# latentnetworks/vimure

Hardware: AMD Instinct MI355X
Metric: CAVI iterations/sec (L=4 N=2000 M=200 K=2 synthetic, mutuality on) (higher is better)
Workload: dtype f64

## Files before the change

### include/vimure_hip.h

```cpp
#ifndef VIMURE_HIP_H
#define VIMURE_HIP_H

#include <stdint.h>

#ifdef __cplusplus
extern "C" {
#endif

typedef struct vmr_ctx* vmr_handle;

enum {
  VMR_OK = 0,
  VMR_EINVAL = -1,
  VMR_EHIP = -2,
  VMR_ENAN = -3,
  VMR_ESTATE = -4
};

enum { VMR_STEP_GAMMA = 0, VMR_STEP_PHI = 1, VMR_STEP_RHO = 2, VMR_STEP_NU = 3 };

enum { VMR_READ_RHO_MAX = 0, VMR_READ_RHO_MEAN = 1, VMR_READ_THRESHOLD = 2 };

enum {
  VMR_KERNEL_GAMMA_MASK = 0,
// ... 157 lines not shown
int vmr_get_geometric(vmr_handle h, double* g_theta, double* g_lambda, double* g_nu, double* g_nu_cache);

int vmr_sync(vmr_handle h);

int vmr_profile(vmr_handle h, int enable);
int vmr_profile_read(vmr_handle h, int kernel_class, double* total_ms, int64_t* launches);

int vmr_kernel_bytes(vmr_handle h, int kernel_class, double* bytes);

int vmr_data_format(vmr_handle h, int* sparse, uint64_t* nnz);

int vmr_mask_format(vmr_handle h, int* lists, uint64_t* listed);

int vmr_sweep_shape(vmr_handle h, int* passes, int* lds_levels, uint64_t* far_reports);

int vmr_generate_y(int device, int L, int N, int K, int C, const double* w, const int32_t* grp, uint64_t seed, uint8_t* Y_dev);
int vmr_generate_x(int device, int L, int N, int M, const uint8_t* Y_dev, const double* lam_dev, const double* theta, double eta,
                   double lambda_diff, uint64_t seed, int self_reporter, uint8_t* X_dev);

const char* vmr_version(void);

#ifdef __cplusplus
}
#endif
#endif
```

### vimure_amd/_lib.py

```python
import ctypes as C
import os

HERE = os.path.dirname(os.path.abspath(__file__))
LIB_PATH = os.environ.get("VMR_LIB", os.path.join(HERE, "libvimure_hip.so"))

VMR_OK, VMR_EINVAL, VMR_EHIP, VMR_ENAN, VMR_ESTATE = 0, -1, -2, -3, -4
STEP_GAMMA, STEP_PHI, STEP_RHO, STEP_NU = 0, 1, 2, 3
KERNEL_GAMMA_MASK, KERNEL_GAMMA_COUNTS, KERNEL_PHI, KERNEL_RHO, KERNEL_ELBO, KERNEL_FINALIZE, KERNEL_RHO_ELBO, KERNEL_RHO_NOSTORE = range(8)
READ_RHO_MAX, READ_RHO_MEAN, READ_THRESHOLD = 0, 1, 2
PPC_NSTAT = 6
TRIAD_NSTAT = 6
TRIAD_NAMES = ["transitive", "cyclic", "two_paths", "triangles_u", "wedges_u", "edges_u"]
EDGE_REPORTED, EDGE_INFERRED = 1, 2
SCORE_RHO1, SCORE_PROB = 0, 1
SCORE_NCONF, SCORE_NSUM, SCORE_MAX_THR = 5, 4, 4096
RT_NCOUNT, RT_NSUM = 7, 3
RT_COUNT_NAMES = ["n_scope", "n_rep", "total", "n_inferred", "hits", "mutual", "n_out"]
RT_SUM_NAMES = ["exp_ties", "exp_hits", "exp_total"]
HO_NSUM, HO_NCOUNT = 4, 4
HO_SUM_NAMES = ["logp", "sq_err", "total", "exp_total"]
HO_COUNT_NAMES = ["n", "n_pos", "n_inf", "n_in_mask"]
RS_REPORTS, RS_OMISSIONS = 1, 2
RS_NSUM, RS_NCOUNT, RS_MAX_EDGES = 4, 4, 4096
RS_SUM_NAMES = ["logp", "sq_err", "total", "exp_total"]
# ... 58 lines not shown
    "vmr_report_scores_size": (C.c_int, [C.c_void_p, C.c_int, C.c_void_p, C.c_void_p, C.c_double, C.c_int, C.c_double, C.POINTER(C.c_uint64)]),
    "vmr_report_scores": (C.c_int, [C.c_void_p, C.c_int, C.c_void_p, C.c_void_p, C.c_double, C.c_int, C.c_double, C.c_int, C.c_void_p]
                          + [C.c_void_p] * 4 + [C.c_uint64] + [C.c_void_p] * 8 + [C.c_int]),
    "vmr_reporter_influence_size": (C.c_int, [C.c_void_p, C.c_int] + [C.c_void_p] * 4 + [C.c_double, C.c_int, C.c_double, C.c_int, C.c_double,
                                              C.POINTER(C.c_uint64)]),
    "vmr_reporter_influence": (C.c_int, [C.c_void_p, C.c_int] + [C.c_void_p] * 4 + [C.c_double, C.c_int, C.c_double, C.c_int, C.c_double,
                                         C.c_int, C.c_void_p] + [C.c_void_p] * 3 + [C.c_uint64] + [C.c_void_p] * 9 + [C.c_int]),
    "vmr_snapshot": (C.c_int, [C.c_void_p]),
    "vmr_restore": (C.c_int, [C.c_void_p]),
    "vmr_profile": (C.c_int, [C.c_void_p, C.c_int]),
    "vmr_profile_read": (C.c_int, [C.c_void_p, C.c_int, _dp, C.POINTER(C.c_int64)]),
    "vmr_kernel_bytes": (C.c_int, [C.c_void_p, C.c_int, _dp]),
    "vmr_data_format": (C.c_int, [C.c_void_p, C.POINTER(C.c_int), C.POINTER(C.c_uint64)]),
    "vmr_mask_format": (C.c_int, [C.c_void_p, C.POINTER(C.c_int), C.POINTER(C.c_uint64)]),
    "vmr_sweep_shape": (C.c_int, [C.c_void_p, C.POINTER(C.c_int), C.POINTER(C.c_int), C.POINTER(C.c_uint64)]),
    "vmr_generate_y": (C.c_int, [C.c_int, C.c_int, C.c_int, C.c_int, C.c_int, C.c_void_p, C.c_void_p, C.c_uint64, C.c_void_p]),
    "vmr_generate_x": (C.c_int, [C.c_int, C.c_int, C.c_int, C.c_int, C.c_void_p, C.c_void_p, C.c_void_p, C.c_double, C.c_double,
                                 C.c_uint64, C.c_int, C.c_void_p]),
    "vmr_version": (C.c_char_p, []),
}

_lib = None


def load():
    global _lib
    if _lib is not None:
        return _lib
    if not os.path.exists(LIB_PATH):
        raise RuntimeError(
# ... 16 lines not shown
```

### vimure_amd/csrc/sorted_lists.hip

```cpp
#include "sweep_sl.h"

__global__ __launch_bounds__(256) void k_sl_keys(const unsigned* __restrict__ cnt, unsigned* __restrict__ keys, unsigned* __restrict__ vals, size_t T) {
  for (size_t t = (size_t)blockIdx.x * 256 + threadIdx.x; t < T; t += (size_t)gridDim.x * 256) { keys[t] = cnt[t]; vals[t] = (unsigned)t; }
}
__global__ __launch_bounds__(256) void k_sl_level_keys(unsigned* __restrict__ keys, const unsigned* __restrict__ rpl, const unsigned* __restrict__ E,
                                                       size_t T, unsigned rows0, int nb) {
  for (size_t t = (size_t)blockIdx.x * 256 + threadIdx.x; t < T; t += (size_t)gridDim.x * 256) {
    const unsigned r0 = rpl[t], n = rpl[t + 1] - r0;
    unsigned n1 = 0;
    for (unsigned r = 0; r < n; ++r) n1 += SL_YM(E[(size_t)r0 + r]) >= rows0 ? 1u : 0u;
    keys[t] = (n << nb) | n1;
  }
}
__global__ __launch_bounds__(256) void k_sl_steps(const unsigned* __restrict__ keys_sorted, const unsigned* __restrict__ vals_sorted,
                                                  unsigned* __restrict__ sz, unsigned* __restrict__ perm, size_t T, size_t NS, int nb) {
  for (size_t q = (size_t)blockIdx.x * 256 + threadIdx.x; q < NS * 64; q += (size_t)gridDim.x * 256) {
    perm[q] = q < T ? vals_sorted[q] : 0xffffffffu;
    if ((q & 63) == 0) sz[q >> 6] = 64u * (keys_sorted[q] >> nb);
  }
  if (blockIdx.x == 0 && threadIdx.x == 0) sz[NS] = 0u;
}
__global__ __launch_bounds__(256) void k_sl_place(const unsigned* __restrict__ perm, const unsigned* __restrict__ rpl ,
                                                  const unsigned* __restrict__ rsl, const unsigned* __restrict__ Ein,
                                                  unsigned* __restrict__ Eout, const unsigned* __restrict__ Ein2, unsigned* __restrict__ Eout2,
// ... 77 lines not shown
  CKS(hipMalloc(&h->perm, (size_t)L * NS * 64 * 4));
  CKS(hipMalloc(&h->sy, (size_t)L * NS * 4));
  size_t tb = 0;
  int bits = 1;
  while (bits < 32 && (1ull << bits) <= (unsigned long long)g.M) ++bits;
  const bool level_keys_ok = !wide && g.mut && 2 * bits <= 30 && !h->opt.no_level_sort;
  CKS(hipcub::DeviceRadixSort::SortPairsDescending(nullptr, tb, keys, keys2, vals, vals2, (int)T, 0, level_keys_ok ? 2 * bits : bits, h->stream));
  CKS(hipMalloc(&tmp, tb ? tb : 8));
  const unsigned tgrid = (unsigned)std::min<size_t>(8192, (T + 255) / 256), sgrid = (unsigned)std::min<size_t>(8192, (NS + 3) / 4);
  if (!etmp_all) {
    unsigned long long nlmax = 0;
    for (int l = 0; l < L; ++l) nlmax = std::max(nlmax, nl[l]);
    CKS(hipMalloc(&etmp, ((size_t)nlmax + 64) * 4));
    if (wide) CKS(hipMalloc(&etmp2, ((size_t)nlmax + 64) * 4));
  }
  unsigned long long off1 = 0;
  for (int l = 0; l < L; ++l) {
    unsigned* rpl = rp + (size_t)l * n;
    unsigned* rsl = h->rs + (size_t)l * (NS + 1);
    const bool by_level = level_keys_ok && (double)nl[l] > (double)SL_PF * (double)T;
    const int nb = by_level ? bits : 0;
    int rc;
    hipLaunchKernelGGL(k_sl_keys, dim3(tgrid), dim3(256), 0, h->stream, rpl, keys, vals, T);
    if (by_level) {
      if ((rc = scan_u32(h, rpl, bsum, n))) { cleanup(); return rc; }
      if (!etmp_all) (*fill)(l, rpl, etmp, etmp2);
      hipLaunchKernelGGL(k_sl_level_keys, dim3(tgrid), dim3(256), 0, h->stream, keys, rpl, etmp_all ? etmp_all + off1 : etmp, T, (unsigned)g.Mp, nb);
    }
    CKS(hipcub::DeviceRadixSort::SortPairsDescending(tmp, tb, keys, keys2, vals, vals2, (int)T, 0, bits + nb, h->stream));
    hipLaunchKernelGGL(k_sl_steps, dim3((unsigned)std::min<size_t>(8192, (NS * 64 + 255) / 256)), dim3(256), 0, h->stream, keys2, vals2, rsl,
                       h->perm + (size_t)l * NS * 64, T, NS, nb);
    CKS(hipGetLastError());
    if ((rc = scan_u32(h, rsl, bsum, NS + 1)) || (!by_level && (rc = scan_u32(h, rpl, bsum, n)))) { cleanup(); return rc; }
    off1 += nl[l];
  }
// ... 52 lines not shown
```

### vimure_amd/csrc/sweep_sl.h

```cpp
#ifndef VMR_SWEEP_SL_H
#define VMR_SWEEP_SL_H

#include "vmr_internal.h"
#include <functional>

#define SL_YM(e) ((e) & 0xfffffu)
#define SL_INR(e) (((e) >> 20) & 1u)
#define SL_X(e) ((e) >> 21)
#define SL_XMAX 2047u
#define SL_YM_ROWS (1u << 20)
#define SL_PF 8
#ifndef SL_PFW
#define SL_PFW 8
#endif
constexpr int sl_pf(int K) { return K <= 2 ? SL_PF : SL_PFW; }
#define SL_SLACK (64 * 64)

struct SlArgs {
  const unsigned* E; const unsigned* rs; const unsigned long long* ebase; const unsigned* perm;
  const unsigned* sy;
  const uint8_t* cls;
  const unsigned* Qt;
  const uint64_t* Rb; const unsigned* rq; const unsigned short* Rm; const unsigned long long* rbase;
  const unsigned* rm2;
// ... 2 lines not shown
  int Gl;
  int do_hist;
  int yt, hc;
  int sum_a;
  double* nu_acc; double* elbo_dev; int commit_nu;
  int nu_stale;
  unsigned long long* det;
  int lp0;
  int farl;
  double* h0s;
  const unsigned* x0p;
  int lv0r;
  const unsigned* Ez;
  int elbo_cur;
  const double* lpd; const double* lpb;
#ifdef SL_DEBUG
  unsigned long long* dbg_t;
#endif
};

struct SlShape { int tpb, yt, hc; size_t smem; };
struct SlUnit { SlArgs a; Geo g; int blk0, nblk; };

#ifndef SL_LIGHT_UPD_K
#define SL_LIGHT_UPD_K 2
#endif
constexpr bool sl_light(int K, bool elbo, bool allfull, bool update) { return !elbo && allfull && (K <= SL_LIGHT_UPD_K || (!update && K <= 4)); }
#ifndef SL_ELBO3_K
#define SL_ELBO3_K 2
#endif
// ... 32 lines not shown
```

### vimure_amd/csrc/sweep_sl.hip

```cpp
#include "sweep_sl.h"

#ifndef VMR_K
#error "compile with -DVMR_K=<number of categories>"
#endif
#ifndef SL_WPE
#define SL_WPE sl_wpe(2, false, true)
#endif

template <int K>
struct StepIn {
  double v[K];
  double w[K];
  unsigned cls, qt, tie;
  unsigned x0;
  unsigned e[sl_pf(K)];
};

template <int R> struct RC { static constexpr int value = R; };
template <class V> __device__ __forceinline__ const V* at_bytes(const V* p, unsigned off) {
  return reinterpret_cast<const V*>(reinterpret_cast<const char*>(p) + off);
}
template <class V> __device__ __forceinline__ V* at_bytes(V* p, unsigned off) {
  return reinterpret_cast<V*>(reinterpret_cast<char*>(p) + off);
}
// ... 1 lines not shown
  double r = __builtin_amdgcn_rcp(d);
  r = fma(fma(-d, r, 1.0), r, r);
  return fma(fma(-d, r, 1.0), r, r);
}
#define SL_INL __attribute__((always_inline))
#ifndef SL_BATCH2
#define SL_BATCH2 8
#endif
template <int K> struct Batch { static constexpr int value = K <= 2 ? SL_BATCH2 : (K <= 4 ? 4 : 2); };

template <int K, bool UPDATE, bool ELBO, bool ALLFULL, bool STORE = true, bool DET = false, bool LPD = false>
__device__ __forceinline__ void sweep_body(const SlArgs& a, const Geo& g, const unsigned bx, const unsigned gx) {
  extern __shared__ __align__(16) unsigned char smem[];
  constexpr int PFK = sl_pf(K);
  constexpr bool LV0 = !UPDATE && !ELBO && !DET;
  constexpr bool LV0R = UPDATE && K >= 3;
  const int tid = threadIdx.x, lane = tid & 63, nthr = (int)blockDim.x;
  const int wv = __builtin_amdgcn_readfirstlane(tid >> 6), nw = nthr >> 6;
  const int Mp = g.Mp;
  const unsigned ytm = UPDATE ? (unsigned)a.yt * (unsigned)Mp : 0u;
  const unsigned hcm = a.do_hist ? (unsigned)a.hc * (unsigned)Mp : 0u;
  size_t off = 0;
  double* F = reinterpret_cast<double*>(smem + off); off += (size_t)ytm * K * 8;
  const int nHc = (int)hcm * K;
  double* Hc = reinterpret_cast<double*>(smem + off); off += (size_t)nHc * 8;
  double* Gth = reinterpret_cast<double*>(smem + off); off += (size_t)Mp * 8;
  double* Lth = reinterpret_cast<double*>(smem + off); off += UPDATE ? (size_t)Mp * 8 : 0;
  double* As = reinterpret_cast<double*>(smem + off); off += a.sum_a ? (size_t)Mp * K * 8 : 0;
  double* wsum = reinterpret_cast<double*>(smem + off); off += (size_t)g.W * 8;
  double* red = reinterpret_cast<double*>(smem + off); off += 16 * 8;
// ... 1 lines not shown
  double* lt = reinterpret_cast<double*>(smem + off); off += ELBO ? 256 * 8 : 0;
  double* EthL = reinterpret_cast<double*>(smem + off); off += a.rq ? (size_t)Mp * 8 : 0;
  const ParOff o = par_off(g.L, g.Mp, g.K);
  const int l = (int)bx / a.Gl, gb = (int)bx - l * a.Gl;
#ifdef SL_DEBUG
  unsigned long long* dbt = a.dbg_t ? a.dbg_t + ((size_t)bx * nw + wv) * 8 : nullptr;
  if (dbt && lane == 0) dbt[0] = wall_clock64();
#endif
  const size_t T = (size_t)g.N * g.N;
  const long long NS = (long long)((T + 63) / 64);
  const double gnu = a.par[o.sc + ((UPDATE || a.elbo_cur) ? SC_G_NU : SC_G_NU_STALE)];
  bool gz = false;
  for (int m = tid; m < Mp; m += nthr) {
    const double gv = a.par[o.G_th + (size_t)l * Mp + m];
    Gth[m] = gv;
    if (LV0 || LV0R) gz = gz || (m < g.M && gv == 0.0);
    if (UPDATE) Lth[m] = a.par[o.l_th + (size_t)l * Mp + m];
  }
  for (int q = tid; q < nHc; q += nthr) Hc[q] = 0.0;
  if (a.sum_a) for (int q = tid; q < Mp * K; q += nthr) As[q] = 0.0;
  if (a.rq) for (int m = tid; m < Mp; m += nthr) EthL[m] = m < g.M ? a.par[o.E_th + (size_t)l * Mp + m] : 0.0;
  if (UPDATE || ELBO) sp_math_tables(xt, lt, tid, nthr, ELBO);
  const double* lut = a.lutg + (size_t)l * g.W * 256;
  for (int w = tid; w < g.W; w += nthr) {
    double v = 0.0;
    for (int n = 0; n < 16; ++n) v += lut[(w * 16 + n) * 16 + 15];
    wsum[w] = v;
  }
  double Ela[K], Gla[K], Lla[K];
#pragma unroll
  for (int k = 0; k < K; ++k) { Ela[k] = a.par[o.E_la + l * K + k]; Gla[k] = a.par[o.G_la + l * K + k]; Lla[k] = a.par[o.l_la + l * K + k]; if (LV0 || LV0R) gz = gz || Gla[k] == 0.0; }
  const double eps = g.eps;
  const double sc_h = DET ? __builtin_amdgcn_ldexp(1.0, g.det_sh) : 0.0;
  const double sc_a = DET ? __builtin_amdgcn_ldexp(1.0, g.det_sha) : 0.0;
  auto fxm = [](double v, double scale) SL_INL -> unsigned long long {
    return (unsigned long long)(__double_as_longlong(fma(v, scale, 6755399441055744.0)) - 0x4338000000000000ll);
  };
  auto lds_add = [&](double* p, double v, double scale) SL_INL {
    if (DET) atomicAdd(reinterpret_cast<unsigned long long*>(p), fxm(v, scale)); else atomicAdd(p, v);
  };
  const float rcp_mp = 1.0f / (float)Mp, hrcp_mp = 0.5f * rcp_mp;
  auto row_level = [&](unsigned ym) SL_INL -> unsigned { return (unsigned)__builtin_fmaf((float)ym, rcp_mp, hrcp_mp); };
  const double lp0_0 = log(1.0 + eps), lp0_k = log(eps);
  double e_lin = 0.0, e_q = 0.0, e_log = 0.0;
  double accF[K], acc0[K];
#pragma unroll
// ... 81 lines not shown
  };

  if (s < NS) {
    ea = rsl[s];
    R = (int)((rsl[s + 1] - ea) >> 6);
    ymax = syl[s];
    fetch_range(sn < NS ? sn : s);
    fetch_tie(P, s);
    fetch_ent(P, ea, RC<PFK>{});
  }
#ifdef SL_DEBUG
  if (dbt && lane == 0) dbt[4] = wall_clock64();
#endif
  __builtin_amdgcn_s_waitcnt(0x0F70);
  bool lv0_off = false;
  if (LV0 || LV0R) lv0_off = __syncthreads_or(gz ? 1 : 0) != 0;
  else __syncthreads();
#ifdef SL_DEBUG
  if (dbt && lane == 0) dbt[5] = wall_clock64();
#endif
  const double gnu_f = a.par[o.sc + (a.nu_stale ? SC_G_NU_STALE : SC_G_NU)];
  if (UPDATE) {
    for (int q = tid; q < (int)ytm; q += nthr) {
      const int y = q / Mp, m = q - y * Mp;
#pragma unroll
      for (int k = 0; k < K; ++k) F[q * K + k] = (m < g.M) ? f_entry(g.mut, Lth[m], Gth[m], Lla[k], Gla[k], gnu_f, y) : 0.0;
    }
    __syncthreads();
  }
  double Tfull = 0.0;
  for (int w = 0; w < g.W; ++w) Tfull += wsum[w];
// ... 128 lines not shown
      if (ELBO) {
#pragma unroll
        for (int u = 0; u < LG; ++u) if (j0 + u < NP) {
          const double term = (double)SL_X(e[j0 + u]) * log_tab(in_[u], lt);
          if (DET) ie_log += det_fx(term, g.det_shr); else e_log += term;
        }
        __builtin_amdgcn_sched_barrier(0);
      }
    }
  };
  auto deficit = [&](unsigned ent, double dfc) SL_INL {
    lds_add(&Hc[SL_YM(ent)], (double)SL_X(ent) * dfc, sc_h);
  };
  auto compute = [&](auto rct, const StepIn<K>& cur, const size_t row0, const bool act, const unsigned ea_c, const int Rr, const unsigned sy_word) SL_INL {
    const unsigned ymax = sy_word & 0xffffu, nf = a.farl ? sy_word >> 16 : 0x7fffffffu;
    const unsigned n1 = (LV0 && a.h0s && !lv0_off) ? sy_word >> 16 : 0x7fffffffu;
    constexpr int RCT = decltype(rct)::value;
    constexpr int NP = RCT < 0 ? PFK : RCT;
    const unsigned cls = cur.cls, qt = cur.qt, tie = cur.tie;
    const unsigned* pe = El + ea_c;
    auto rounds = [&](auto gbc, auto&& use, const int Rr) SL_INL {
      constexpr int GB = decltype(gbc)::value;
      unsigned rg[PFK];
#pragma unroll
      for (int i = 0; i < PFK; ++i) rg[i] = i < Rr ? cur.e[i] : 0u;
      for (int j0 = 0; j0 < Rr; j0 += PFK) {
#pragma unroll
        for (int gi = 0; gi < PFK; gi += GB) {
          unsigned c[GB];
#pragma unroll
          for (int u = 0; u < GB; ++u) {
// ... 144 lines not shown
      if (irr && lane == 0) tick[1] = 1u;
      if (!ELBO && a.do_hist == 1 && act && (ALLFULL || cls == 1u)) {
#pragma unroll
        for (int k = 0; k < K; ++k) { if (DET) iaccF[k] += fxm(r[k], sc_a); else accF[k] += r[k]; }
      }
      if (!ALLFULL && !ELBO && a.sum_a) add_lists(tie, act && cls == 2u, r);
    }
    if (ELBO) {
#pragma unroll
      for (int k = 0; k < K; ++k) { const double ek = exp_tab(r[k], xt); er[0] = fma(ek, Gla[k], er[0]); er[1] += ek; }
    }
#ifdef SL_DEBUG
    if (g.dbg & 32) {} else
#endif
    if (a.do_hist || ELBO) {
      if (RCT >= 0) {
        walk2_near(cur.e, RC<NP>{}, r, er);
        if (irr) {
#pragma unroll
          for (int j = 0; j < NP; ++j) deficit(cur.e[j], dfc);
        }
      } else {
        const bool skip0 = LV0 && a.x0p != nullptr && a.do_hist == 1 && n1 != 0x7fffffffu && !irr;
        const int Rw = skip0 ? min(Rr, (int)n1) : Rr;
        double sx0 = skip0 ? (double)cur.x0 : 0.0;
        rounds(RC<1>{}, [&](const unsigned (&c1)[1], const unsigned j) SL_INL {
          const unsigned c = c1[0], ym = SL_YM(c), x = SL_X(c);
          const bool far_round = j < nf && lim2 != 0xffffffffu;
          const bool fr = far_round && ym >= hcm;
          const double dx = (double)x;
          if (LV0 && a.do_hist && j >= n1) {
            sx0 += dx;
            if (irr) lds_add(&Hc[ym], dx * dfc, sc_h);
          } else if (a.do_hist) {
            if (!fr) {
              if (!(skip0 && ym < (unsigned)Mp)) {
#pragma unroll
                for (int k = 1; k < K; ++k) lds_add(&Hc[(unsigned)k * hcm + ym], dx * r[k], sc_h);
              }
              if (irr) lds_add(&Hc[ym], dx * dfc, sc_h);
            }
            if (far_round && !a.farl && __any(fr)) {
              if (fr && x != 0u) {
                if (DET) {
                  unsigned long long* d0 = a.det;
                  asm volatile("" : "+s"(d0));
                  unsigned long long* d = d0 + (size_t)l * g.Y * Mp * K + (size_t)ym * K;
#pragma unroll
                  for (int k = 1; k < K; ++k) atomicAdd(&d[k], fxm((double)x * r[k], sc_h));
                  if (dfc != 0.0) atomicAdd(&d[0], fxm((double)x * dfc, sc_h));
                } else {
                  double* d = Hl + (size_t)ym * K;
#pragma unroll
                  for (int k = 1; k < K; ++k) atomicAdd(&d[k], (double)x * r[k]);
                  if (dfc != 0.0) atomicAdd(&d[0], (double)x * dfc);
                }
              }
              asm volatile("" ::: "memory");
            }
          }
          if (ELBO) { const double term = (double)x * log_tab(elbo_inner(c, er), lt); if (DET) ie_log += det_fx(term, g.det_shr); else e_log += term; }
        }, Rw);
        if (LV0 && a.h0s && a.do_hist == 1 && act) {
#pragma unroll
          for (int k = 1; k < K; ++k) acc0[k] = fma(r[k], sx0, acc0[k]);
        }
      }
    }
    if (ELBO && act) {
      double sr = 0.0, se = 0.0, en = 0.0;
#pragma unroll
      for (int k = 0; k < K; ++k) {
        sr += r[k]; se += r[k] * Ela[k];
        en += r[k] * cur.v[k] - r[k] * log_tab(r[k] + eps, lt);
      }
      if (DET) { ie_lin += det_fx(en - se * Tt, g.det_shr); if (Ql) ie_q += det_fx(sr * (double)qt, g.det_shr); }
      else { e_lin += en - se * Tt; if (Ql) e_q += sr * (double)qt; }
    }
// ... 44 lines not shown
      case 3: run(RC<3>{}); break;
      case 4: run(RC<4>{}); break;
      case 5: run(RC<5>{}); break;
      case 6: run(RC<6>{}); break;
      case 7: run(RC<7>{}); break;
      default: run(RC<8>{}); break;
    }
  }

#ifdef SL_DEBUG
  if (dbt && lane == 0) dbt[2] = wall_clock64();
#endif
  const bool nu_here = a.nu_acc && a.do_hist == 1;
  if (nu_here) asm volatile("s_waitcnt vmcnt(0)" ::: "memory");
  __syncthreads();
  if (nu_here) {
    double a0p = 0.0;
    for (int q = (tick[1] ? 0 : (int)hcm) + tid; q < nHc; q += nthr) {
      const double v = DET ? det_back(reinterpret_cast<const unsigned long long*>(Hc)[q], g.det_sh) : Hc[q];
      if (v != 0.0) {
        const int k = q / (int)hcm;
        const unsigned ym = (unsigned)(q - k * (int)hcm);
        a0p += ((k ? w2_at(ym, k) : 0.0) - w2_at(ym, 0)) * v;
      }
    }
    a0p = block_sum_n(a0p, red);
    if (tid == 0) {
      if (DET) atomicAdd(&det_R()[4], det_fx(a0p, g.det_sh)); else atomicAdd(&a.nu_acc[0], a0p);
    }
  }
// ... 267 lines not shown
```

### vimure_amd/csrc/vimure_hip.hip

```cpp
#include "vmr_internal.h"
#include "sweep_sl.h"
#include "sweep_gen.h"
#include "sample_draw.h"

thread_local std::string g_create_err;



template <int SH>
__device__ __forceinline__ unsigned nz_flags16(uint4 v) {
  const unsigned M = 0x7f7f7f7fu;
  unsigned t0 = ((v.x & M) + M) | v.x, t1 = ((v.y & M) + M) | v.y;
  unsigned t2 = ((v.z & M) + M) | v.z, t3 = ((v.w & M) + M) | v.w;
  unsigned f = (t0 >> (7 - SH)) & (0x01010101u << SH);
  f |= (t1 >> (6 - SH)) & (0x02020202u << SH);
  f |= (t2 >> (5 - SH)) & (0x04040404u << SH);
  f |= (t3 >> (4 - SH)) & (0x08080808u << SH);
  return f;
}
__device__ __forceinline__ void flag_pos(int bit, int& chunk, int& byte) {
  const int lo = bit & 31;
  chunk = ((bit >> 5) << 1) | ((lo >> 2) & 1);
  byte = ((lo & 3) << 2) | (lo >> 3);
}
// ... 1556 lines not shown
  if (update && !g.two_pass) n += shmem_hc(g);
  if (elbo) n += (size_t)g.Mp * 8 + (size_t)g.nt * 4;
  return n + 16;
}

#define SP_LDS_MAX (160 * 1024)

static SlShape sl_shape(const vmr_ctx* h, bool update, bool elbo, bool hist) {
  const Geo& g = h->g;
  SlShape s{std::max(64, std::min((update || elbo) ? h->sp_tpb : h->st_tpb, sl_tpb_max(g.K, elbo, h->all_full != 0, update)) & ~63), update ? g.yt : 0, hist ? g.hc : 0, 0};
  auto bytes = [&]() { return sl_smem(g, s.yt, s.hc, update, elbo, hist); };
  while (bytes() > SP_LDS_MAX && (s.yt > 0 || s.hc > 0)) { if (s.yt >= s.hc && s.yt > 0) --s.yt; else --s.hc; }
  s.smem = bytes();
  return s;
}
static SlArgs sl_args(const vmr_ctx* h, const SlShape& sh, int do_hist, int sum_a = 0) {
  return SlArgs{h->E, h->rs, h->ebase, h->perm, h->sy, h->cls_p, h->Qt_p, h->Rb, h->rq, h->Rm, h->rbase, h->rm2, h->rho, h->logpr, h->par, h->slotR,
                h->lutg, h->Hg, h->slotF, h->slotA, 1, do_hist, sh.yt, sh.hc, sum_a, nullptr, nullptr, 0, 0, nullptr, h->lp0 ? 1 : 0, h->g.farl, (do_hist == 1 && h->g.two_pass && sh.hc >= 1) ? h->h0s : nullptr, (do_hist == 1 && h->g.two_pass && sh.hc >= 1 && h->h0s) ? h->x0p : nullptr,
                (h->h0s && h->g.two_pass && !h->opt.no_lv0r) ? 1 : 0, h->E + h->n_slots, 0, h->lpd, h->lpb};
}
static int sl_launch(vmr_ctx* h, int mode, const SlShape& sh, SlArgs& a) {
  sl_launch_fn fn = vmr_sl_launcher(h->g.K);
  if (!fn) return fail(h, VMR_EINVAL, "this build of libvimure_hip.so holds no sweep kernel for this K");
  return fn(h, mode, sh, a);
}

#ifdef VMR_DEV
#define DISPATCH_K(K_, ...)                         \
  switch (K_) {                                     \
    case 2: { constexpr int KK = 2; __VA_ARGS__; } break; \
    default: break;                                 \
  }
#else
#define DISPATCH_K(K_, ...)                         \
// ... 12 lines not shown
  switch (PF_) {                                                      \
    case 4: { constexpr int PP = 4; DISPATCH_K(K_, __VA_ARGS__); } break;   \
    case 8: { constexpr int PP = 8; DISPATCH_K(K_, __VA_ARGS__); } break;   \
    default: { constexpr int PP = 12; DISPATCH_K(K_, __VA_ARGS__); } break; \
  }



__global__ __launch_bounds__(256) void k_stat_slots(const unsigned* __restrict__ rsl, const unsigned* __restrict__ syl, size_t NS, unsigned long long* __restrict__ out) {
  unsigned long long v = 0;
  for (size_t s = (size_t)blockIdx.x * 256 + threadIdx.x; s < NS; s += (size_t)gridDim.x * 256) {
    const unsigned R = (rsl[s + 1] - rsl[s]) >> 6, n1 = syl[s] >> 16;
    v += 64ull * (unsigned long long)min(R, n1);
  }
  if (v) atomicAdd(out, v);
}
__global__ __launch_bounds__(256) void k_far_first(unsigned* __restrict__ E, const unsigned* __restrict__ rsl, unsigned* __restrict__ syl, size_t NS, unsigned rows_near,
                                                   unsigned* __restrict__ x0) {
  const int lane = threadIdx.x & 63;
  for (size_t s = (size_t)blockIdx.x * 4 + (threadIdx.x >> 6); s < NS; s += (size_t)gridDim.x * 4) {
    const unsigned ea = rsl[s], R = (rsl[s + 1] - ea) >> 6;
    unsigned* col = E + (size_t)ea + lane;
    unsigned f = 0;
    unsigned xs = 0;
    for (unsigned r = 0; r < R; ++r) {
      const unsigned e = col[(size_t)r * 64];
      if (e != 0u && SL_YM(e) >= rows_near) {
        if (f != r) { const unsigned o = col[(size_t)f * 64]; col[(size_t)f * 64] = e; col[(size_t)r * 64] = o; }
        ++f;
      } else xs += SL_X(e);
// ... 383 lines not shown
  dim3 blk(TPB);
  int rc = VMR_OK;
  if (mode != 2 && !h->h_zero) {
    if (g.fuse_full) HIPCHK(h, hipMemsetAsync(h->slotF, 0, (size_t)g.L * NSLOT * g.K * 8, h->stream));
    if (!g.two_pass) HIPCHK(h, hipMemsetAsync(h->Hg, 0, (size_t)g.L * NH * g.Y * g.Mp * g.K * 8, h->stream));
  }
  if (mode != 2) h->h_zero = false;
  const bool nu_in_pass = h->sparse && g.mut && mode != 2 && (commit_nu || raw_nu);
  if (mode == 2 && (rc = ensure_rho(h))) return rc;
  if (h->sparse) {
    const int do_hist = (mode != 2 && !g.two_pass) ? 1 : 0;
    const int sum_a = (g.ml && do_hist) ? 1 : 0;
    if (mode != 2) h->a_valid = false;
    if (sum_a) { if ((rc = begin_sum_a(h, h->stream))) return rc; h->a_valid = true; }
    const SlShape shs = sl_shape(h, mode != 2, mode != 0, do_hist != 0);
    SlArgs as = sl_args(h, shs, do_hist, sum_a);
    if (nu_in_pass && do_hist) { as.nu_acc = h->nu_acc; as.elbo_dev = h->elbo_dev; as.commit_nu = commit_nu ? 1 : 0; }
    as.det = g.det ? h->det_buf : nullptr;
    const bool lazy = !store && mode == 0 && do_hist && (nu_in_pass ? commit_nu : !g.mut) && g.fuse_full && (h->n_partial == 0 || g.ml) &&
                      !g.farl && !h->opt.always_store_rho;
    {
      Prof p(h, lazy ? VMR_KERNEL_RHO_NOSTORE : mode == 2 ? VMR_KERNEL_ELBO : mode == 1 ? VMR_KERNEL_RHO_ELBO : VMR_KERNEL_RHO);
      if ((rc = sl_launch(h, lazy ? 4 : mode, shs, as))) return rc;
    }
    if (mode != 2) h->rho_stale = lazy;
    if (g.farl && do_hist && (rc = launch_far(h, 0, nu_in_pass ? (commit_nu ? 1 : 0) : -1))) return rc;
    if ((rc = det_fold(h))) return rc;
  } else {
    Prof p(h, mode == 2 ? VMR_KERNEL_ELBO : mode == 1 ? VMR_KERNEL_RHO_ELBO : VMR_KERNEL_RHO);
#define LRHO(MUT_, UPD_, ELB_)                                                                  \
  DISPATCH_KP(g.K, g.pf, if ((rc = grid_per_layer(h, k_rho<KK, MUT_, UPD_, ELB_, PP>, sm, &a.Gl))) return rc; \
// ... 65 lines not shown
  memset(&o, 0, sizeof o);
  auto set = [](const char* n) { return getenv(n) != nullptr; };
  auto num = [](const char* n, int dflt) { const char* e = getenv(n); return e ? atoi(e) : dflt; };
  if (const char* f = getenv("VMR_FORMAT")) o.format = !strcmp(f, "dense") ? 1 : !strcmp(f, "sparse") ? 2 : 0;
  o.deterministic = num("VMR_DETERMINISTIC", 0) != 0;
  o.graph = num("VMR_GRAPH", 0) != 0;
  o.debug = num("VMR_DEBUG", 0);
  o.levels = num("VMR_LEVELS", 64);
  o.two_pass = num("VMR_TWO_PASS", 0);
  o.farl = num("VMR_FARL", 0);
  o.yt = set("VMR_YT") ? std::max(0, num("VMR_YT", 0)) : -1;
  o.hc = set("VMR_HC") ? std::max(0, num("VMR_HC", 0)) : -1;
  o.tpb = num("VMR_TPB", 0);
  o.st_tpb = num("VMR_ST_TPB", 0);
  o.no_level0 = set("VMR_NO_LEVEL0");
  o.no_x0 = set("VMR_NO_X0");
  o.no_lv0r = set("VMR_NO_LV0R");
  o.no_level_sort = set("VMR_NO_LEVEL_SORT");
  o.no_rlists = set("VMR_NO_RLISTS");
  o.no_rm2 = set("VMR_NO_RM2");
  o.no_lp0 = set("VMR_NO_LP0");
  o.no_lpd = set("VMR_NO_LPD");
  o.always_store_rho = set("VMR_ALWAYS_STORE_RHO");
  o.debug_lazy_rho = set("VMR_DEBUG_LAZY_RHO");
  o.gen_hsum = num("VMR_GEN_HSUM", 0);
  o.gen_no_lds_h = set("VMR_GEN_NO_LDS_H");
  o.gen_dbg = num("VMR_GEN_DBG", 0);
  o.netstats_chunk = std::max(0, num("VMR_NETSTATS_CHUNK", 0));
  o.batch_fg = set("VMR_BATCH_FG") ? std::max(1, std::min(FG_G, num("VMR_BATCH_FG", 0))) : 0;
  if (const char* t = getenv("VMR_DEBUG_TIMES")) snprintf(o.debug_times, sizeof o.debug_times, "%s", t);
// ... 355 lines not shown
      if (h->x0p) {
        unsigned long long* ss = nullptr;
        CK(hipMalloc(&ss, 8));
        CK(hipMemsetAsync(ss, 0, 8, h->stream));
        for (int l = 0; l < L; ++l)
          hipLaunchKernelGGL(k_stat_slots, dim3(256), dim3(256), 0, h->stream, h->rs + (size_t)l * (NS_ + 1), h->sy + (size_t)l * NS_, NS_, ss);
        hipError_t es = hipMemcpyAsync(&h->stat_slots, ss, 8, hipMemcpyDeviceToHost, h->stream);
        if (es == hipSuccess) es = hipStreamSynchronize(h->stream);
        (void)hipFree(ss);
        CK(es);
      }
      const size_t n0 = (size_t)L * NSLOT * K + L;
      CK(hipMalloc(&h->h0s, n0 * 8));
      CK(hipMemsetAsync(h->h0s, 0, n0 * 8, h->stream));
    }
    if (g.farl) {
      bool same = g.hc >= 1 && g.hc < g.Y;
      for (int v : {0, 3}) same = same && sl_shape(h, v != 3, false, true).hc == g.hc;
      h->elbo_split = sl_shape(h, true, true, true).hc != g.hc || sl_shape(h, true, true, true).yt != g.yt;
      if (!same) g.farl = 0;
      else { int rcf = build_far_lists(h); if (rcf) return rcf; }
    }
  } else {
    if (shmem_rho(g, true, false) > 80000) {
      g.two_pass = 1;
      while (g.hc > 0 && shmem_hist(g) > 160000) --g.hc;
    }
    need = std::max(shmem_rho(g, true, true), shmem_hist(g));
  }
  if (need > (size_t)prop.sharedMemPerBlock && need > 160 * 1024) {
// ... 816 lines not shown
        return t;
      };
      if (total(per) > cap_wgs) {
        long long p2 = per;
        while (p2 < 512 && total(p2) > cap_wgs) p2 += std::max<long long>(1, p2 / 16);
        if (total(p2) <= cap_wgs) per = p2;
      }
    }
    std::vector<SlUnit> su(act.size());
    std::vector<int> map;
    size_t smem = 0;
    for (size_t i = 0; i < act.size(); ++i) {
      vmr_ctx* h = hs[act[i]];
      const Geo& g = h->g;
      const SlShape sh = sl_shape(h, m != 2, m == 1, true);
      SlArgs a = sl_args(h, sh, 1, g.ml ? 1 : 0);
      a.elbo_dev = bt.be + (size_t)act[i] * 8;
      if (g.mut && m != 2) { a.nu_acc = h->nu_acc; a.commit_nu = 1; }
      const long long NS = ((long long)g.N * g.N + 63) / 64;
      a.Gl = (int)std::max<long long>(1, std::min<long long>(4096, (NS + nw * per - 1) / (nw * per)));
      su[i].a = a; su[i].g = g; su[i].blk0 = (int)map.size(); su[i].nblk = g.L * a.Gl;
      map.insert(map.end(), (size_t)su[i].nblk, (int)i);
      smem = std::max(smem, sh.smem);
    }
    HIPCHK(h0, hipMemcpyAsync(bt.su[m], su.data(), su.size() * sizeof(SlUnit), hipMemcpyHostToDevice, st));
    HIPCHK(h0, hipMemcpyAsync(bt.smap[m], map.data(), map.size() * sizeof(int), hipMemcpyHostToDevice, st));
    HIPCHK(h0, hipStreamSynchronize(st));
    bt.nb[m] = (int)map.size(); bt.tpb[m] = tpb; bt.smem[m] = smem;
  }
  bt.fsm = 0;
  {
// ... 434 lines not shown
int vmr_mask_format(vmr_handle h, int* lists, uint64_t* listed) {
  if (!h) return VMR_EINVAL;
  if (lists) *lists = h->rq ? 1 : 0;
  if (listed) *listed = h->n_rm;
  return VMR_OK;
}

int vmr_sweep_shape(vmr_handle h, int* passes, int* lds_levels, uint64_t* far_reports) {
  if (!h) return VMR_EINVAL;
  if (passes) *passes = h->g.two_pass ? 2 : 1;
  if (lds_levels) *lds_levels = h->g.gen ? 0 : h->g.hc;
  if (far_reports) *far_reports = (h->g.farl && !h->far_off.empty()) ? h->far_off.back() : 0ull;
  return VMR_OK;
}

int vmr_kernel_bytes(vmr_handle h, int kernel_class, double* bytes) {
  if (!h || !bytes) return VMR_EINVAL;
  const Geo& g = h->g;
  const double V = (double)g.L * g.N * g.N * g.M;
  const double SX = V, SR = V / 8.0, Srho = 8.0 * g.L * (double)g.N * g.N * g.K;
  if (h->sparse) {
    const double ties = (double)g.L * g.N * g.N;
    const double E = (g.wide ? 8.0 : 4.0) * (double)h->nnz, RP = 4.0 * (ties / 64.0 + g.L);
    const double mask = h->all_full ? 0.0 : ties + (h->rq ? 4.0 * ties + 2.0 * (double)h->n_rm : (double)h->n_partial * g.W * 8.0);
    const double Q = g.mut ? 4.0 * ties : 0.0;
    const double Slp = h->lpd ? 8.0 * ties : Srho;
    switch (kernel_class) {
      case VMR_KERNEL_GAMMA_MASK: *bytes = ties + (h->rq ? 4.0 * ties + 2.0 * (double)h->n_rm : (double)h->n_partial * g.W * 8.0) + Srho; break;
      case VMR_KERNEL_GAMMA_COUNTS:
        *bytes = ((h->x0p && g.two_pass) ? 4.0 * (double)h->stat_slots + 4.0 * ties : E) + RP + Srho;
// ... 23 lines not shown
```

### vimure_amd/csrc/vmr_internal.h

```cpp
#ifndef VMR_INTERNAL_H
#define VMR_INTERNAL_H
#include <hip/hip_runtime.h>
#include <hipcub/hipcub.hpp>
#include <stdint.h>
#include <stdio.h>
#include <string.h>
#include <math.h>
#include <stdlib.h>
#include <string>
#include <vector>
#include <utility>
#include <algorithm>
#include <chrono>
#include <type_traits>

#include "vimure_hip.h"

#define VMR_VERSION "vimure_hip 0.1 (gfx950)"
#define TPB 256
#ifndef VMR_LB_COUNTS
#define VMR_LB_COUNTS 4
#endif
#ifndef VMR_LB_RHO
#define VMR_LB_RHO 3
// ... 36 lines not shown
};
#define DET_SH2 30
__device__ __forceinline__ unsigned long long det_fx(double v, int sh) { return (unsigned long long)__double2ll_rn(ldexp(v, sh)); }
__device__ __forceinline__ double det_back(unsigned long long u, int sh) { return ldexp((double)(long long)u, -sh); }

#define NSLOT 8

struct VmrOpts {
  int format;
  bool deterministic, graph;
  int debug, levels;
  int two_pass, farl;
  int yt, hc;
  int tpb, st_tpb;
  bool no_level0, no_x0, no_lv0r, no_level_sort, no_rlists, no_rm2, no_lp0, no_lpd;
  bool always_store_rho, debug_lazy_rho;
  int gen_hsum;
  bool gen_no_lds_h;
  int gen_dbg;
  int batch_fg;
  int netstats_chunk;
  char debug_times[256];
};

struct vmr_ctx {
  Geo g;
  VmrOpts opt;
  int device;
  hipStream_t stream;
  hipStream_t stream2 = nullptr;
// ... 15 lines not shown
  int st_tpb = 256;
  unsigned* Qt = nullptr;
  unsigned long long* ebase = nullptr;
  unsigned long long nnz = 0;
  unsigned long long n_slots = 0;
  int all_full = 0;
  unsigned* perm = nullptr;
  unsigned* sy = nullptr;
  unsigned* far_pos = nullptr;
  unsigned* far_ent = nullptr;
  unsigned long long* far_base = nullptr;
  std::vector<unsigned long long> far_off;
  double* h0s = nullptr;
  unsigned long long stat_slots = 0;
  unsigned* x0p = nullptr;
  bool elbo_split = false;
  uint8_t* cls_p = nullptr;
  unsigned* Qt_p = nullptr;
  double* nat = nullptr;
  unsigned* rq = nullptr;
  unsigned short* Rm = nullptr;
  unsigned long long* rbase = nullptr;
  unsigned long long n_rm = 0;
  unsigned rm_maxrow = 0;
  unsigned* rm2 = nullptr;
  int coo_mb = 13;
  unsigned long long* sumx = nullptr;
  double *rho = nullptr, *logpr = nullptr;
  double *lpd = nullptr, *lpb = nullptr;
  double* par = nullptr;
// ... 297 lines not shown
```

### vimure_amd/engine.py

```python
import ctypes as C

import numpy as np

from . import _lib


class EngineError(RuntimeError):
    pass


class EdgeTableArgumentError(EngineError, ValueError):
    """An argument `edge_table` / `edge_table_size` refuse (VMR_EINVAL): a method that gives no categories, an empty or
    unknown selection, outputs shorter than the table."""


class ScoreArgumentError(EngineError, ValueError):
    """An argument `score_truth` refuses (VMR_EINVAL): an unknown score, thresholds that are not finite, that decrease or that
    are too many, a ground truth of another shape, no output asked for."""


class ReporterTableArgumentError(EngineError, ValueError):
    """An argument `reporter_table` refuses (VMR_EINVAL): a method that gives no categories, a layer out of range, no output
    asked for."""

# ... 863 lines not shown
    def data_format(self):
        sp, nnz = C.c_int(), C.c_uint64()
        self._check(self.lib.vmr_data_format(self._h, C.byref(sp), C.byref(nnz)))
        return ("sparse" if sp.value else "dense"), int(nnz.value)

    def mask_format(self):
        li, n = C.c_int(), C.c_uint64()
        self._check(self.lib.vmr_mask_format(self._h, C.byref(li), C.byref(n)))
        return ("lists" if li.value else "words"), int(n.value)

    def sweep_shape(self):
        p, lv, n = C.c_int(), C.c_int(), C.c_uint64()
        self._check(self.lib.vmr_sweep_shape(self._h, C.byref(p), C.byref(lv), C.byref(n)))
        return int(p.value), int(lv.value), int(n.value)

    def profile(self, enable=True):
        self._check(self.lib.vmr_profile(self._h, int(enable)))

    def profile_read(self):
        out = {}
        for i, name in enumerate(_lib.KERNEL_NAMES):
            ms, n, b = C.c_double(), C.c_int64(), C.c_double()
            self._check(self.lib.vmr_profile_read(self._h, i, C.byref(ms), C.byref(n)))
            self._check(self.lib.vmr_kernel_bytes(self._h, i, C.byref(b)))
            out[name] = {"ms": ms.value, "launches": n.value, "bytes_per_launch": b.value}
        return out
```

Baseline: 5970.

## Collapse level-0 histogram updates in single-pass mutuality sweep via per-layer scaling

Extends the level-0 shortcut to the update sweep for K=2 in the one-pass (non-two-pass, non-far) mutuality path. Entries at the zero level are summed into a per-thread scalar instead of being atomically added to LDS one by one. After the block reduction, each column's histogram gets a precomputed per-column count times a scale factor. At setup it forces level-keyed sorting of the lists and reorders entries so level-0 entries come last, which adds init work and a new code branch in compute.

Measured after the change: 5935. Within noise of the previous version (-0.6%).

```diff
diff --git a/include/vimure_hip.h b/include/vimure_hip.h
--- a/include/vimure_hip.h
+++ b/include/vimure_hip.h
@@ -195,6 +195,8 @@
 
 int vmr_sweep_shape(vmr_handle h, int* passes, int* lds_levels, uint64_t* far_reports);
 
+int vmr_level0_rounds(vmr_handle h, uint64_t* rounds, uint64_t* level0_rounds);
+
 int vmr_generate_y(int device, int L, int N, int K, int C, const double* w, const int32_t* grp, uint64_t seed, uint8_t* Y_dev);
 int vmr_generate_x(int device, int L, int N, int M, const uint8_t* Y_dev, const double* lam_dev, const double* theta, double eta,
                    double lambda_diff, uint64_t seed, int self_reporter, uint8_t* X_dev);
diff --git a/vimure_amd/_lib.py b/vimure_amd/_lib.py
--- a/vimure_amd/_lib.py
+++ b/vimure_amd/_lib.py
@@ -96,6 +96,7 @@
     "vmr_data_format": (C.c_int, [C.c_void_p, C.POINTER(C.c_int), C.POINTER(C.c_uint64)]),
     "vmr_mask_format": (C.c_int, [C.c_void_p, C.POINTER(C.c_int), C.POINTER(C.c_uint64)]),
     "vmr_sweep_shape": (C.c_int, [C.c_void_p, C.POINTER(C.c_int), C.POINTER(C.c_int), C.POINTER(C.c_uint64)]),
+    "vmr_level0_rounds": (C.c_int, [C.c_void_p, C.POINTER(C.c_uint64), C.POINTER(C.c_uint64)]),
     "vmr_generate_y": (C.c_int, [C.c_int, C.c_int, C.c_int, C.c_int, C.c_int, C.c_void_p, C.c_void_p, C.c_uint64, C.c_void_p]),
     "vmr_generate_x": (C.c_int, [C.c_int, C.c_int, C.c_int, C.c_int, C.c_void_p, C.c_void_p, C.c_void_p, C.c_double, C.c_double,
                                  C.c_uint64, C.c_int, C.c_void_p]),
diff --git a/vimure_amd/csrc/sorted_lists.hip b/vimure_amd/csrc/sorted_lists.hip
--- a/vimure_amd/csrc/sorted_lists.hip
+++ b/vimure_amd/csrc/sorted_lists.hip
@@ -115,11 +115,14 @@
     CKS(hipMalloc(&etmp, ((size_t)nlmax + 64) * 4));
     if (wide) CKS(hipMalloc(&etmp2, ((size_t)nlmax + 64) * 4));
   }
+  const VmrOpts& o = h->opt;
+  h->lv0_cand = level_keys_ok && !g.gen && g.K == 2 && !g.det && g.Y > 1 && !o.no_level0 && !o.no_lpd &&
+                (o.level0_one_pass >= 0 ? o.level0_one_pass != 0 : g.N > 1024);
   unsigned long long off1 = 0;
   for (int l = 0; l < L; ++l) {
     unsigned* rpl = rp + (size_t)l * n;
     unsigned* rsl = h->rs + (size_t)l * (NS + 1);
-    const bool by_level = level_keys_ok && (double)nl[l] > (double)SL_PF * (double)T;
+    const bool by_level = level_keys_ok && (h->lv0_cand || (double)nl[l] > (double)SL_PF * (double)T);
     const int nb = by_level ? bits : 0;
     int rc;
     hipLaunchKernelGGL(k_sl_keys, dim3(tgrid), dim3(256), 0, h->stream, rpl, keys, vals, T);
diff --git a/vimure_amd/csrc/sweep_sl.h b/vimure_amd/csrc/sweep_sl.h
--- a/vimure_amd/csrc/sweep_sl.h
+++ b/vimure_amd/csrc/sweep_sl.h
@@ -40,6 +40,7 @@
   const unsigned* Ez;
   int elbo_cur;
   const double* lpd; const double* lpb;
+  const double* c0;
 #ifdef SL_DEBUG
   unsigned long long* dbg_t;
 #endif
diff --git a/vimure_amd/csrc/sweep_sl.hip b/vimure_amd/csrc/sweep_sl.hip
--- a/vimure_amd/csrc/sweep_sl.hip
+++ b/vimure_amd/csrc/sweep_sl.hip
@@ -39,6 +39,7 @@
   extern __shared__ __align__(16) unsigned char smem[];
   constexpr int PFK = sl_pf(K);
   constexpr bool LV0 = !UPDATE && !ELBO && !DET;
+  constexpr bool LV0U = K == 2 && UPDATE && !ELBO && !DET && LPD;
   constexpr bool LV0R = UPDATE && K >= 3;
   const int tid = threadIdx.x, lane = tid & 63, nthr = (int)blockDim.x;
   const int wv = __builtin_amdgcn_readfirstlane(tid >> 6), nw = nthr >> 6;
@@ -70,7 +71,7 @@
   for (int m = tid; m < Mp; m += nthr) {
     const double gv = a.par[o.G_th + (size_t)l * Mp + m];
     Gth[m] = gv;
-    if (LV0 || LV0R) gz = gz || (m < g.M && gv == 0.0);
+    if (LV0 || LV0R || LV0U) gz = gz || (m < g.M && gv == 0.0);
     if (UPDATE) Lth[m] = a.par[o.l_th + (size_t)l * Mp + m];
   }
   for (int q = tid; q < nHc; q += nthr) Hc[q] = 0.0;
@@ -85,7 +86,7 @@
   }
   double Ela[K], Gla[K], Lla[K];
 #pragma unroll
-  for (int k = 0; k < K; ++k) { Ela[k] = a.par[o.E_la + l * K + k]; Gla[k] = a.par[o.G_la + l * K + k]; Lla[k] = a.par[o.l_la + l * K + k]; if (LV0 || LV0R) gz = gz || Gla[k] == 0.0; }
+  for (int k = 0; k < K; ++k) { Ela[k] = a.par[o.E_la + l * K + k]; Gla[k] = a.par[o.G_la + l * K + k]; Lla[k] = a.par[o.l_la + l * K + k]; if (LV0 || LV0R || LV0U) gz = gz || Gla[k] == 0.0; }
   const double eps = g.eps;
   const double sc_h = DET ? __builtin_amdgcn_ldexp(1.0, g.det_sh) : 0.0;
   const double sc_a = DET ? __builtin_amdgcn_ldexp(1.0, g.det_sha) : 0.0;
@@ -197,7 +198,7 @@
 #endif
   __builtin_amdgcn_s_waitcnt(0x0F70);
   bool lv0_off = false;
-  if (LV0 || LV0R) lv0_off = __syncthreads_or(gz ? 1 : 0) != 0;
+  if (LV0 || LV0R || LV0U) lv0_off = __syncthreads_or(gz ? 1 : 0) != 0;
   else __syncthreads();
 #ifdef SL_DEBUG
   if (dbt && lane == 0) dbt[5] = wall_clock64();
@@ -356,7 +357,7 @@
   };
   auto compute = [&](auto rct, const StepIn<K>& cur, const size_t row0, const bool act, const unsigned ea_c, const int Rr, const unsigned sy_word) SL_INL {
     const unsigned ymax = sy_word & 0xffffu, nf = a.farl ? sy_word >> 16 : 0x7fffffffu;
-    const unsigned n1 = (LV0 && a.h0s && !lv0_off) ? sy_word >> 16 : 0x7fffffffu;
+    const unsigned n1 = ((LV0 || LV0U) && a.h0s && !lv0_off) ? sy_word >> 16 : 0x7fffffffu;
     constexpr int RCT = decltype(rct)::value;
     constexpr int NP = RCT < 0 ? PFK : RCT;
     const unsigned cls = cur.cls, qt = cur.qt, tie = cur.tie;
@@ -531,7 +532,18 @@
     if (g.dbg & 32) {} else
 #endif
     if (a.do_hist || ELBO) {
-      if (RCT >= 0) {
+      if (RCT >= 0 && LV0U && a.do_hist && n1 < (unsigned)NP && !irr) {
+        unsigned sx0i = 0u;
+#pragma unroll
+        for (int j = 0; j < NP; ++j) {
+          unsigned ej = cur.e[j];
+          asm volatile("" : "+v"(ej));
+          if ((unsigned)j < n1) lds_add(&Hc[hcm + SL_YM(ej)], (double)SL_X(ej) * r[1], sc_h);
+          else sx0i += SL_X(ej);
+        }
+        const double sx0 = (double)sx0i;
+        if (act) acc0[1] = fma(r[1], sx0, acc0[1]);
+      } else if (RCT >= 0) {
         walk2_near(cur.e, RC<NP>{}, r, er);
         if (irr) {
 #pragma unroll
@@ -540,15 +552,16 @@
       } else {
         const bool skip0 = LV0 && a.x0p != nullptr && a.do_hist == 1 && n1 != 0x7fffffffu && !irr;
         const int Rw = skip0 ? min(Rr, (int)n1) : Rr;
+        const unsigned n1w = (LV0U && irr) ? 0x7fffffffu : n1;
         double sx0 = skip0 ? (double)cur.x0 : 0.0;
         rounds(RC<1>{}, [&](const unsigned (&c1)[1], const unsigned j) SL_INL {
           const unsigned c = c1[0], ym = SL_YM(c), x = SL_X(c);
           const bool far_round = j < nf && lim2 != 0xffffffffu;
           const bool fr = far_round && ym >= hcm;
           const double dx = (double)x;
-          if (LV0 && a.do_hist && j >= n1) {
+          if ((LV0 || LV0U) && a.do_hist && j >= n1w) {
             sx0 += dx;
-            if (irr) lds_add(&Hc[ym], dx * dfc, sc_h);
+            if (!LV0U && irr) lds_add(&Hc[ym], dx * dfc, sc_h);
           } else if (a.do_hist) {
             if (!fr) {
               if (!(skip0 && ym < (unsigned)Mp)) {
@@ -578,7 +591,7 @@
           }
           if (ELBO) { const double term = (double)x * log_tab(elbo_inner(c, er), lt); if (DET) ie_log += det_fx(term, g.det_shr); else e_log += term; }
         }, Rw);
-        if (LV0 && a.h0s && a.do_hist == 1 && act) {
+        if ((LV0 || LV0U) && a.h0s && a.do_hist == 1 && act) {
 #pragma unroll
           for (int k = 1; k < K; ++k) acc0[k] = fma(r[k], sx0, acc0[k]);
         }
@@ -653,6 +666,17 @@
   const bool nu_here = a.nu_acc && a.do_hist == 1;
   if (nu_here) asm volatile("s_waitcnt vmcnt(0)" ::: "memory");
   __syncthreads();
+  if (LV0U && a.c0 && a.h0s && a.do_hist == 1) {
+    const double s1 = block_sum_n(acc0[1], red);
+    if (tid == 0) { const double tot = a.h0s[(size_t)g.L * NSLOT * K + l]; red[0] = tot > 0.0 ? s1 / tot : 0.0; }
+    __syncthreads();
+    const double sk = red[0];
+    if (sk != 0.0) {
+      const double* C0 = a.c0 + (size_t)l * g.Y * Mp;
+      for (int m = tid; m < g.M; m += nthr) { const double c = C0[m]; if (c != 0.0) Hc[hcm + (unsigned)m] += c * sk; }
+    }
+    __syncthreads();
+  }
   if (nu_here) {
     double a0p = 0.0;
     for (int q = (tick[1] ? 0 : (int)hcm) + tid; q < nHc; q += nthr) {
diff --git a/vimure_amd/csrc/vimure_hip.hip b/vimure_amd/csrc/vimure_hip.hip
--- a/vimure_amd/csrc/vimure_hip.hip
+++ b/vimure_amd/csrc/vimure_hip.hip
@@ -1594,10 +1594,11 @@
   s.smem = bytes();
   return s;
 }
-static SlArgs sl_args(const vmr_ctx* h, const SlShape& sh, int do_hist, int sum_a = 0) {
+static SlArgs sl_args(const vmr_ctx* h, const SlShape& sh, int do_hist, int sum_a = 0, bool update = false) {
+  const bool l0u = update && do_hist == 1 && h->lv0_one && sh.hc >= 1;
   return SlArgs{h->E, h->rs, h->ebase, h->perm, h->sy, h->cls_p, h->Qt_p, h->Rb, h->rq, h->Rm, h->rbase, h->rm2, h->rho, h->logpr, h->par, h->slotR,
-                h->lutg, h->Hg, h->slotF, h->slotA, 1, do_hist, sh.yt, sh.hc, sum_a, nullptr, nullptr, 0, 0, nullptr, h->lp0 ? 1 : 0, h->g.farl, (do_hist == 1 && h->g.two_pass && sh.hc >= 1) ? h->h0s : nullptr, (do_hist == 1 && h->g.two_pass && sh.hc >= 1 && h->h0s) ? h->x0p : nullptr,
-                (h->h0s && h->g.two_pass && !h->opt.no_lv0r) ? 1 : 0, h->E + h->n_slots, 0, h->lpd, h->lpb};
+                h->lutg, h->Hg, h->slotF, h->slotA, 1, do_hist, sh.yt, sh.hc, sum_a, nullptr, nullptr, 0, 0, nullptr, h->lp0 ? 1 : 0, h->g.farl, ((do_hist == 1 && h->g.two_pass && sh.hc >= 1) || l0u) ? h->h0s : nullptr, (do_hist == 1 && h->g.two_pass && sh.hc >= 1 && h->h0s) ? h->x0p : nullptr,
+                (h->h0s && h->g.two_pass && !h->opt.no_lv0r) ? 1 : 0, h->E + h->n_slots, 0, h->lpd, h->lpb, l0u ? h->Cg : nullptr};
 }
 static int sl_launch(vmr_ctx* h, int mode, const SlShape& sh, SlArgs& a) {
   sl_launch_fn fn = vmr_sl_launcher(h->g.K);
@@ -1640,6 +1641,15 @@
     v += 64ull * (unsigned long long)min(R, n1);
   }
   if (v) atomicAdd(out, v);
+}
+__global__ __launch_bounds__(256) void k_level0_rounds(const unsigned* __restrict__ rsl, const unsigned* __restrict__ syl, size_t NS, unsigned long long* __restrict__ out) {
+  unsigned long long v = 0, v0 = 0;
+  for (size_t s = (size_t)blockIdx.x * 256 + threadIdx.x; s < NS; s += (size_t)gridDim.x * 256) {
+    const unsigned R = (rsl[s + 1] - rsl[s]) >> 6, n1 = syl[s] >> 16;
+    v += R; v0 += R - min(R, n1);
+  }
+  if (v) atomicAdd(&out[0], v);
+  if (v0) atomicAdd(&out[1], v0);
 }
 __global__ __launch_bounds__(256) void k_far_first(unsigned* __restrict__ E, const unsigned* __restrict__ rsl, unsigned* __restrict__ syl, size_t NS, unsigned rows_near,
                                                    unsigned* __restrict__ x0) {
@@ -2053,7 +2063,7 @@
     if (mode != 2) h->a_valid = false;
     if (sum_a) { if ((rc = begin_sum_a(h, h->stream))) return rc; h->a_valid = true; }
     const SlShape shs = sl_shape(h, mode != 2, mode != 0, do_hist != 0);
-    SlArgs as = sl_args(h, shs, do_hist, sum_a);
+    SlArgs as = sl_args(h, shs, do_hist, sum_a, mode != 2);
     if (nu_in_pass && do_hist) { as.nu_acc = h->nu_acc; as.elbo_dev = h->elbo_dev; as.commit_nu = commit_nu ? 1 : 0; }
     as.det = g.det ? h->det_buf : nullptr;
     const bool lazy = !store && mode == 0 && do_hist && (nu_in_pass ? commit_nu : !g.mut) && g.fuse_full && (h->n_partial == 0 || g.ml) &&
@@ -2149,6 +2159,7 @@
   o.tpb = num("VMR_TPB", 0);
   o.st_tpb = num("VMR_ST_TPB", 0);
   o.no_level0 = set("VMR_NO_LEVEL0");
+  o.level0_one_pass = set("VMR_LEVEL0_ONE_PASS") ? (num("VMR_LEVEL0_ONE_PASS", 0) != 0 ? 1 : 0) : -1;
   o.no_x0 = set("VMR_NO_X0");
   o.no_lv0r = set("VMR_NO_LV0R");
   o.no_level_sort = set("VMR_NO_LEVEL_SORT");
@@ -2534,6 +2545,28 @@
       CK(hipMalloc(&h->h0s, n0 * 8));
       CK(hipMemsetAsync(h->h0s, 0, n0 * 8, h->stream));
     }
+    if (h->lv0_cand && !g.two_pass && !g.farl && g.mut && !g.det && g.Y > 1 && g.hc >= 1 && sl_shape(h, true, false, true).hc >= 1) {
+      const size_t T_ = (size_t)g.N * g.N, NS_ = (T_ + 63) / 64;
+      std::vector<unsigned long long> eb(L);
+      CK(hipMemcpy(eb.data(), h->ebase, (size_t)L * 8, hipMemcpyDeviceToHost));
+      unsigned long long* rr = nullptr;
+      CK(hipMalloc(&rr, 16));
+      CK(hipMemsetAsync(rr, 0, 16, h->stream));
+      for (int l = 0; l < L; ++l) {
+        hipLaunchKernelGGL(k_far_first, dim3((unsigned)std::min<size_t>(8192, (NS_ + 3) / 4)), dim3(256), 0, h->stream, h->E + eb[l], h->rs + (size_t)l * (NS_ + 1),
+                           h->sy + (size_t)l * NS_, NS_, (unsigned)g.Mp, (unsigned*)nullptr);
+        hipLaunchKernelGGL(k_level0_rounds, dim3(256), dim3(256), 0, h->stream, h->rs + (size_t)l * (NS_ + 1), h->sy + (size_t)l * NS_, NS_, rr);
+      }
+      hipError_t er_ = hipGetLastError();
+      if (er_ == hipSuccess) er_ = hipMemcpyAsync(h->l0_rounds, rr, 16, hipMemcpyDeviceToHost, h->stream);
+      if (er_ == hipSuccess) er_ = hipStreamSynchronize(h->stream);
+      (void)hipFree(rr);
+      CK(er_);
+      const size_t n0 = (size_t)L * NSLOT * K + L;
+      CK(hipMalloc(&h->h0s, n0 * 8));
+      CK(hipMemsetAsync(h->h0s, 0, n0 * 8, h->stream));
+      h->lv0_one = true;
+    }
     if (g.farl) {
       bool same = g.hc >= 1 && g.hc < g.Y;
       for (int v : {0, 3}) same = same && sl_shape(h, v != 3, false, true).hc == g.hc;
@@ -3380,7 +3413,7 @@
       vmr_ctx* h = hs[act[i]];
       const Geo& g = h->g;
       const SlShape sh = sl_shape(h, m != 2, m == 1, true);
-      SlArgs a = sl_args(h, sh, 1, g.ml ? 1 : 0);
+      SlArgs a = sl_args(h, sh, 1, g.ml ? 1 : 0, m != 2);
       a.elbo_dev = bt.be + (size_t)act[i] * 8;
       if (g.mut && m != 2) { a.nu_acc = h->nu_acc; a.commit_nu = 1; }
       const long long NS = ((long long)g.N * g.N + 63) / 64;
@@ -3845,6 +3878,13 @@
   return VMR_OK;
 }
 
+int vmr_level0_rounds(vmr_handle h, uint64_t* rounds, uint64_t* level0_rounds) {
+  if (!h) return VMR_EINVAL;
+  if (rounds) *rounds = h->lv0_one ? h->l0_rounds[0] : (h->sparse ? h->n_slots / 64ull : 0ull);
+  if (level0_rounds) *level0_rounds = h->lv0_one ? h->l0_rounds[1] : 0ull;
+  return VMR_OK;
+}
+
 int vmr_kernel_bytes(vmr_handle h, int kernel_class, double* bytes) {
   if (!h || !bytes) return VMR_EINVAL;
   const Geo& g = h->g;
diff --git a/vimure_amd/csrc/vmr_internal.h b/vimure_amd/csrc/vmr_internal.h
--- a/vimure_amd/csrc/vmr_internal.h
+++ b/vimure_amd/csrc/vmr_internal.h
@@ -74,6 +74,7 @@
   int yt, hc;
   int tpb, st_tpb;
   bool no_level0, no_x0, no_lv0r, no_level_sort, no_rlists, no_rm2, no_lp0, no_lpd;
+  int level0_one_pass;
   bool always_store_rho, debug_lazy_rho;
   int gen_hsum;
   bool gen_no_lds_h;
@@ -119,6 +120,9 @@
   double* h0s = nullptr;
   unsigned long long stat_slots = 0;
   unsigned* x0p = nullptr;
+  bool lv0_cand = false;
+  bool lv0_one = false;
+  unsigned long long l0_rounds[2] = {0, 0};
   bool elbo_split = false;
   uint8_t* cls_p = nullptr;
   unsigned* Qt_p = nullptr;
diff --git a/vimure_amd/engine.py b/vimure_amd/engine.py
--- a/vimure_amd/engine.py
+++ b/vimure_amd/engine.py
@@ -901,6 +901,11 @@
         self._check(self.lib.vmr_sweep_shape(self._h, C.byref(p), C.byref(lv), C.byref(n)))
         return int(p.value), int(lv.value), int(n.value)
 
+    def level0_rounds(self):
+        r, r0 = C.c_uint64(), C.c_uint64()
+        self._check(self.lib.vmr_level0_rounds(self._h, C.byref(r), C.byref(r0)))
+        return int(r.value), int(r0.value)
+
     def profile(self, enable=True):
         self._check(self.lib.vmr_profile(self._h, int(enable)))
 
```
